# kyungminn/PBHC

Hardware: AMD Instinct MI355X
Metric: env-steps/s (obs+reward+PPO update), 4096 G1 envs @1/2/4/8 MI355X (higher is better)
Workload: dtype f32; 1 GPU; 4096 envs/GPU, G1 23-DoF, single reference motion g1_walk_45cms (122 frames), v1 env (LeggedRobotMotionTracking) + MHPPO, 24 steps/iter, 5 epochs x 4 minibatches; replay sim-stub tensors resident in HBM; envs_per_gpu=4096, global_envs=4096, num_steps_per_env=24, parallelism=dp1

## Files before the change

### pbhc_amd/csrc/pbhc_gemm.hip

```cpp
#include <hip/hip_runtime.h>
#include <stdint.h>
#include <stdio.h>

#include "../../include/pbhc_hip.h"

extern thread_local char g_pbhc_err[512];
#define GEMM_FAIL(code, ...) do { snprintf(g_pbhc_err, sizeof(g_pbhc_err), __VA_ARGS__); return (code); } while (0)
#define GEMM_ARG(cond) do { if (!(cond)) GEMM_FAIL(PBHC_EINVAL, "%s: argument check failed: %s", __func__, #cond); } while (0)
#define GEMM_HIP(expr) do { hipError_t e_ = (expr); if (e_ != hipSuccess) GEMM_FAIL(PBHC_EHIP, "%s: %s: %s", __func__, #expr, hipGetErrorString(e_)); } while (0)

typedef float f32x16 __attribute__((ext_vector_type(16)));
typedef float f32x4 __attribute__((ext_vector_type(4)));
typedef float f32x2 __attribute__((ext_vector_type(2)));

#define GEMM_T 256

#ifndef PBHC_GEMM_LIBM_EXP
#define GEMM_EXP(x) __builtin_amdgcn_exp2f((x) * 1.44269504088896341f)
#define GEMM_RCP(x) __builtin_amdgcn_rcpf(x)
#else
#define GEMM_EXP(x) expf(x)
#define GEMM_RCP(x) (1.0f / (x))
#endif
__device__ __forceinline__ float gemm_act(int act, float v) {
// ... 309 lines not shown
    } else {
      prow_or_kr = 2 * (p - A_PIECES) + (lane >> 5);
      c = ((lane & 31) - 8 * ((prow_or_kr >> 2) & 1)) & 31;
    }
  };
  unsigned voff[LPW];
#pragma unroll
  for (int i = 0; i < LPW; ++i) {
    int q, c; bool kc, isA;
    piece_geom(i, q, c, kc, isA);
    if (kc) {
      const int grow = min((isA ? row0 : col0) + q, (isA ? M : N) - 1);
      voff[i] = ((unsigned)grow * (unsigned)(isA ? lda : K) + 4u * c) * 4u;
    } else {
      voff[i] = ((unsigned)q * (unsigned)N + (unsigned)min(col0 + 4 * c, N - 4)) * 4u;
    }
  }
  auto issue = [&](int st, auto slot_c) {
    constexpr int SLOT = decltype(slot_c)::value;
    const int k0 = st * BK;
    if (tail && st == nk - 1) {
#pragma unroll
      for (int i = 0; i < LPW; ++i) {
        const int p = (wave + 4 * i) % PIECES;
        int q, c; bool kc, isA;
        piece_geom(i, q, c, kc, isA);
        const float* g;
        if (kc) {
          const int grow = min((isA ? row0 : col0) + q, (isA ? M : N) - 1);
          const float* rowbase = (isA ? A : B) + (size_t)grow * (isA ? lda : K);
          const int gk = k0 + 4 * c;
          g = gk + 4 <= K ? rowbase + gk : gk < K ? rowbase + (K - 4) : g_gemm_zeros;
        } else {
          g = k0 + q < K ? B + (size_t)(k0 + q) * N + min(col0 + 4 * c, N - 4) : g_gemm_zeros;
        }
        glds16(g, &lds[SLOT * STAGE + p * 256]);
      }
    } else {
      const char* sA = reinterpret_cast<const char*>(A + k0);
      const char* sB = reinterpret_cast<const char*>(MODE == 0 ? B + k0 : B + (size_t)k0 * N);
#pragma unroll
      for (int i = 0; i < LPW; ++i) {
        const int p = (wave + 4 * i) % PIECES;
        const char* sbase = p < A_PIECES ? sA : sB;
        glds16_sv(sbase, voff[i], &lds[SLOT * STAGE + p * 256]);
      }
    }
  };

  f32x16 acc[TM][TN];
#pragma unroll
  for (int j = 0; j < TN; ++j) {
    const int colj = col0 + (wn * TN + j) * 32 + r;
    const float bj = (MODE == 0 && bias && colj < N) ? bias[colj] : 0.0f;
#pragma unroll
    for (int i = 0; i < TM; ++i)
#pragma unroll
      for (int e = 0; e < 16; ++e) acc[i][j][e] = bj;
  }

  const int sw_r = BK == 16 ? (r >> 2) & 3 : (r >> 1) & 7;
  int fa[BK / 8], fb[MODE == 0 ? BK / 8 : TN];
#pragma unroll
  for (int k8 = 0; k8 < BK / 8; ++k8) {
    fa[k8] = (wm * TM * 32 + r) * BK + 4 * ((2 * k8 + kk) ^ sw_r);
    if (MODE == 0) fb[k8] = A_STAGE + (wn * TN * 32 + r) * BK + 4 * ((2 * k8 + kk) ^ sw_r);
  }
  if (MODE == 1) {
#pragma unroll
    for (int j = 0; j < TN; ++j) fb[j] = A_STAGE + 4 * kk * BN + (((wn * TN + j) * 32 + r + 32 * kk) & 127);
  }

  auto stage_body = [&](auto slot_c, int kb) {
    constexpr int SLOT = decltype(slot_c)::value;
    if (kb + NS - 2 < nk) wait_vmcnt<(NS - 2) * LPW>(); else wait_vmcnt<0>();
    lds_barrier_raw();
    if (kb + NS - 1 < nk && !(dbg & 1)) issue(kb + NS - 1, IC<(SLOT + NS - 1) % NS>{});
    if (tail && kb == nk - 1 && (K & 3)) {
      const int rem = K & 3, cst = (K - ktail0) >> 2;
      const int nrows = MODE == 0 ? BM + BN : BM;
      for (int t = tid; t < nrows; t += GEMM_T) {
        const int sw = BK == 16 ? (t >> 2) & 3 : (t >> 1) & 7;
        f32x4* q = reinterpret_cast<f32x4*>(&lds[SLOT * STAGE + t * BK + 4 * (cst ^ sw)]);
        const f32x4 o = *q;
        f32x4 n;
        n[0] = rem == 1 ? o[3] : rem == 2 ? o[2] : o[1];
        n[1] = rem == 1 ? 0.0f : rem == 2 ? o[3] : o[2];
        n[2] = rem == 3 ? o[3] : 0.0f;
        n[3] = 0.0f;
        *q = n;
      }
      lds_barrier_raw();
    }
    f32x4 a[2][TM], b[2][TN];
    auto read_frags = [&](int k8, f32x4 (&af)[TM], f32x4 (&bf)[TN]) {
#pragma unroll
      for (int i = 0; i < TM; ++i) af[i] = *reinterpret_cast<const f32x4*>(&lds[SLOT * STAGE + i * 32 * BK + fa[k8]]);
#pragma unroll
      for (int j = 0; j < TN; ++j) {
        if (MODE == 0) {
          bf[j] = *reinterpret_cast<const f32x4*>(&lds[SLOT * STAGE + j * 32 * BK + fb[k8]]);
        } else {
#pragma unroll
          for (int s = 0; s < 4; ++s) bf[j][s] = lds[SLOT * STAGE + (k8 * 8 + s) * BN + fb[j]];
        }
      }
    };
    read_frags(0, a[0], b[0]);
#pragma unroll
    for (int k8 = 0; k8 < BK / 8; ++k8) {
      if (k8 + 1 < BK / 8) read_frags(k8 + 1, a[(k8 + 1) & 1], b[(k8 + 1) & 1]);
      __builtin_amdgcn_sched_barrier(0);
#pragma unroll
      for (int s = 0; s < 4; ++s)
#pragma unroll
        for (int i = 0; i < TM; ++i)
#pragma unroll
          for (int j = 0; j < TN; ++j) acc[i][j] = __builtin_amdgcn_mfma_f32_32x32x2f32(a[k8 & 1][i][s], b[k8 & 1][j][s], acc[i][j], 0, 0, 0);
    }
  };

  if (0 < nk) issue(0, IC<0>{});
  if (NS > 2 && 1 < nk) issue(1, IC<1 % NS>{});
  if (NS > 3 && 2 < nk) issue(2, IC<2 % NS>{});
  for (int kb = 0; kb < nk; kb += NS) {
    stage_body(IC<0>{}, kb);
    if (kb + 1 < nk) stage_body(IC<1 % NS>{}, kb + 1);
    if (NS > 2 && kb + 2 < nk) stage_body(IC<2 % NS>{}, kb + 2);
    if (NS > 3 && kb + 3 < nk) stage_body(IC<3 % NS>{}, kb + 3);
  }

  if ((dbg & 16) && acc[0][0][0] != 12345.678f) return;
  constexpr int CS = BN + 4;
  constexpr bool CAN_FUSE_OUT = MODE == 0 && BM == 32 && BN == 128;
  const bool fuse_out = CAN_FUSE_OUT && fo.out != nullptr;
  f32x4 wo[3];
  if (CAN_FUSE_OUT && fuse_out) {
#pragma unroll
    for (int q = 0; q < 3; ++q) {
      const int ch = tid + GEMM_T * q;
      const int n = ch >> 5;
      wo[q] = n < fo.no ? reinterpret_cast<const F4U*>(fo.w + (size_t)n * 128 + 4 * (ch & 31))->v : f32x4{0.f, 0.f, 0.f, 0.f};
    }
  }
  lds_barrier_raw();
  if (CAN_FUSE_OUT && fuse_out) {
#pragma unroll
    for (int q = 0; q < 4; ++q) {
      const int ch = tid + GEMM_T * q;
      const int n = ch >> 5;
      f32x4 v = q < 3 ? wo[q < 3 ? q : 0] : f32x4{0.f, 0.f, 0.f, 0.f};
      if (q == 3 && n < fo.no) v = reinterpret_cast<const F4U*>(fo.w + (size_t)n * 128 + 4 * (ch & 31))->v;
      *reinterpret_cast<f32x4*>(&lds[BM * CS + n * CS + 4 * (ch & 31)]) = v;
    }
  }
#pragma unroll
  for (int i = 0; i < TM; ++i)
#pragma unroll
    for (int j = 0; j < TN; ++j)
#pragma unroll
      for (int e = 0; e < 16; ++e)
        lds[((wm * TM + i) * 32 + 8 * (e >> 2) + 4 * kk + (e & 3)) * CS + (wn * TN + j) * 32 + r] = acc[i][j][e];
  lds_barrier_raw();
  {
    constexpr int RP = GEMM_T / (BN / 4);
    constexpr int NP = BM / RP;
    const int c4 = (tid % (BN / 4)) * 4, rr = tid / (BN / 4);
    const int col = col0 + c4;
    const bool vec = (N & 3) == 0;
    const bool cok = vec ? col < N : col < N;
    float csum[4] = {0.f, 0.f, 0.f, 0.f};
    f32x4 sv[NP];
    if (MODE == 1 && act) {
#pragma unroll
      for (int p = 0; p < NP; ++p) {
        const int row = row0 + p * RP + rr;
        sv[p] = f32x4{0.f, 0.f, 0.f, 0.f};
        if (row < M && cok) {
          const float* sp = S + (size_t)row * N + col;
          if (vec) sv[p] = reinterpret_cast<const F4U*>(sp)->v;
          else {
#pragma unroll
            for (int q = 0; q < 4; ++q) if (col + q < N) sv[p][q] = sp[q];
          }
        }
      }
    }
    auto row_pass = [&](auto act_c, auto vec_c) {
      constexpr int ACT = decltype(act_c)::value;
      constexpr bool VEC = (decltype(vec_c)::value & 1) != 0;
      constexpr bool INTERIOR = (decltype(vec_c)::value & 2) != 0;
#pragma unroll
    for (int p = 0; p < NP; ++p) {
      const int row = row0 + p * RP + rr;
      f32x4 v = *reinterpret_cast<const f32x4*>(&lds[(p * RP + rr) * CS + c4]);
      const bool ok = INTERIOR || (row < M && cok);
      if (MODE == 0) {
        if (Pre && ok) {
          float* pp = Pre + (size_t)row * ldc + col;
          if (VEC) reinterpret_cast<F4U*>(pp)->v = v;
          else {
#pragma unroll
            for (int q = 0; q < 4; ++q) if (col + q < N) pp[q] = v[q];
          }
        }
        v = gemm_act4<ACT>(v);
        if (CAN_FUSE_OUT && fuse_out) *reinterpret_cast<f32x4*>(&lds[(p * RP + rr) * CS + c4]) = v;
      } else if (ACT) {
        v = gemm_mul_grad4<ACT>(v, sv[p]);
      }
      if (ok && !((dbg & 2) && v[0] != 12345.678f)) {
        float* cp = Cout + (size_t)row * ldc + col;
        if (VEC && (dbg & 4)) __builtin_nontemporal_store(v, &reinterpret_cast<F4U*>(cp)->v);
        else if (VEC) reinterpret_cast<F4U*>(cp)->v = v;
        else {
#pragma unroll
          for (int q = 0; q < 4; ++q) if (col + q < N) cp[q] = v[q];
        }
        if (MODE == 1) {
#pragma unroll
          for (int q = 0; q < 4; ++q) csum[q] += v[q];
        }
      }
    }
    };
    const bool interior = row0 + BM <= M && col0 + BN <= N;
    if (vec && interior) {
      if (act == 1) row_pass(IC<1>{}, IC<3>{}); else if (act == 2) row_pass(IC<2>{}, IC<3>{}); else if (act == 3) row_pass(IC<3>{}, IC<3>{}); else row_pass(IC<0>{}, IC<3>{});
    } else if (vec) {
      if (act == 1) row_pass(IC<1>{}, IC<1>{}); else if (act == 2) row_pass(IC<2>{}, IC<1>{}); else if (act == 3) row_pass(IC<3>{}, IC<1>{}); else row_pass(IC<0>{}, IC<1>{});
    } else {
      if (act == 1) row_pass(IC<1>{}, IC<0>{}); else if (act == 2) row_pass(IC<2>{}, IC<0>{}); else if (act == 3) row_pass(IC<3>{}, IC<0>{}); else row_pass(IC<0>{}, IC<0>{});
    }
    if ((dbg & 8) && threadIdx.x == 0 && blockIdx.x == gridDim.x / 2) {
      __builtin_amdgcn_s_waitcnt(0);
      Cout[0] = (float)(clock64() - dbg_c0);
      Cout[1] = (float)(wall_clock64() - dbg_w0);
    }
    if constexpr (CAN_FUSE_OUT) {
      if (fuse_out) {
        lds_barrier_raw();
        f32x16 o;
#pragma unroll
        for (int e = 0; e < 16; ++e) o[e] = 0.0f;
#pragma unroll
        for (int k8 = 0; k8 < 4; ++k8) {
          const f32x4 ya = *reinterpret_cast<const f32x4*>(&lds[r * CS + 32 * wave + 8 * k8 + 4 * kk]);
          const f32x4 wb = *reinterpret_cast<const f32x4*>(&lds[BM * CS + r * CS + 32 * wave + 8 * k8 + 4 * kk]);
#pragma unroll
          for (int s = 0; s < 4; ++s) o = __builtin_amdgcn_mfma_f32_32x32x2f32(ya[s], wb[s], o, 0, 0, 0);
        }
        lds_barrier_raw();
#pragma unroll
        for (int e = 0; e < 16; ++e) lds[wave * (32 * 33) + (8 * (e >> 2) + 4 * kk + (e & 3)) * 33 + r] = o[e];
        lds_barrier_raw();
        const int m = tid >> 3, q0 = tid & 7;
        if (row0 + m < M) {
#pragma unroll
          for (int j = 0; j < 4; ++j) {
            const int n = q0 + 8 * j;
            if (n < fo.no) {
              float t = lds[m * 33 + n];
#pragma unroll
              for (int w = 1; w < 4; ++w) t += lds[w * (32 * 33) + m * 33 + n];
              fo.out[(size_t)(row0 + m) * fo.no + n] = t + (fo.b ? fo.b[n] : 0.0f);
            }
          }
        }
      }
    }
    if (MODE == 1 && part) {
      lds_barrier_raw();
      float* red = lds;
#pragma unroll
      for (int q = 0; q < 4; ++q) red[rr * BN + c4 + q] = csum[q];
      lds_barrier_raw();
      for (int c = tid; c < BN; c += GEMM_T) {
        float t = 0.0f;
#pragma unroll
        for (int w = 0; w < RP; ++w) t += red[w * BN + c];
        if (col0 + c < N) part[(size_t)tile_m * N + col0 + c] = t;
      }
    }
  }
}

template <int MODE, int WM, int WN, int TM, int TN, int BK, int NS>
__global__ __launch_bounds__(GEMM_T, 2) void k_gemm2(const float* __restrict__ A, const float* __restrict__ B, const float* __restrict__ bias,
                                                      const float* __restrict__ S, float* __restrict__ Cout, float* __restrict__ Pre, float* __restrict__ part,
                                                      int M, int N, int K, int act, int tiles_n, int dbg, int lda, int ldc, long long a_batch, long long c_batch,
                                                      GemmOutLayer fo) {
  const size_t ao = (size_t)blockIdx.y * a_batch, co = (size_t)blockIdx.y * c_batch;
  const Gemm2Args g{A + ao, B, bias, S, Cout + co, Pre ? Pre + co : nullptr, part, M, N, K, act, tiles_n, dbg, lda, ldc, fo};
  gemm2_tile<MODE, WM, WN, TM, TN, BK, NS>(g, blockIdx.x, gridDim.x);
}

template <int MODE, int WM, int WN, int TM, int TN, int BK, int NS>
__global__ __launch_bounds__(GEMM_T, 2) void k_gemm2_pair(Gemm2Args g0, Gemm2Args g1, int n0) {
  const bool first = (int)blockIdx.x < n0;
  const Gemm2Args g = first ? g0 : g1;
  gemm2_tile<MODE, WM, WN, TM, TN, BK, NS>(g, first ? blockIdx.x : blockIdx.x - n0, first ? n0 : gridDim.x - n0);
}

#define WG_BK 32
#define WG_BM 128
#define WG_BN 128
__global__ __launch_bounds__(GEMM_T, 2) void k_wgrad(const float* __restrict__ dY, const float* __restrict__ X, float* __restrict__ part,
                                                      int N, int K, int stages_total, int tiles_k, int tiles, int P) {
  constexpr int A_STAGE = WG_BK * WG_BM, STAGE = WG_BK * (WG_BM + WG_BN);
  constexpr int A_PIECES = A_STAGE / 256, PIECES = STAGE / 256, LPW = PIECES / 4;
  extern __shared__ __attribute__((aligned(16))) float lds[];
  int tile, p_idx;
  if ((P & 7) == 0) { const int xcd = blockIdx.x & 7, slot = blockIdx.x >> 3; p_idx = xcd + 8 * (slot / tiles); tile = slot - (slot / tiles) * tiles; }
  else { p_idx = blockIdx.x / tiles; tile = blockIdx.x - p_idx * tiles; }
  const int tile_n = tile / tiles_k, tile_k = tile - tile_n * tiles_k;
  const int n0 = tile_n * WG_BM, k0c = tile_k * WG_BN;
  const int tid = threadIdx.x, lane = tid & 63;
  const int wave = __builtin_amdgcn_readfirstlane(tid >> 6);
  const int wm = wave >> 1, wn = wave & 1;
  const int r = lane & 31, kk = lane >> 5;
  const int st0 = (int)((long long)p_idx * stages_total / P), st1 = (int)((long long)(p_idx + 1) * stages_total / P);
  const int nk = st1 - st0;
  const float* dYp = dY + (size_t)st0 * WG_BK * N;
  const float* Xp = X + (size_t)st0 * WG_BK * K;

  unsigned voff[LPW];
#pragma unroll
  for (int i = 0; i < LPW; ++i) {
    const int p = wave + 4 * i;
    const bool isA = p < A_PIECES;
    const int row = (isA ? p : p - A_PIECES) * 2 + (lane >> 5);
    const int c = lane & 31;
    const int col = isA ? min(n0 + 4 * c, N - 4) : min(k0c + 4 * c, K - 4);
    voff[i] = ((unsigned)row * (unsigned)(isA ? N : K) + (unsigned)col) * 4u;
  }
  auto issue = [&](int st, auto slot_c) {
    constexpr int SLOT = decltype(slot_c)::value;
    const char* sA = reinterpret_cast<const char*>(dYp + (size_t)st * WG_BK * N);
    const char* sB = reinterpret_cast<const char*>(Xp + (size_t)st * WG_BK * K);
#pragma unroll
    for (int i = 0; i < LPW; ++i) {
      const int p = wave + 4 * i;
      glds16_sv(p < A_PIECES ? sA : sB, voff[i], &lds[SLOT * STAGE + p * 256]);
    }
  };

  f32x16 acc[2][2];
#pragma unroll
  for (int q = 0; q < 2; ++q)
#pragma unroll
    for (int p = 0; p < 2; ++p)
#pragma unroll
      for (int e = 0; e < 16; ++e) acc[q][p][e] = 0.0f;
  const int fa = kk * WG_BM + wm * 64 + 2 * r;
  const int fb = A_STAGE + kk * WG_BN + wn * 64 + 2 * r;

  auto stage_body = [&](auto slot_c, int kb) {
    constexpr int SLOT = decltype(slot_c)::value;
    wait_vmcnt<0>();
    lds_barrier_raw();
    if (kb + 1 < nk) issue(kb + 1, IC<(SLOT + 1) % 2>{});
    f32x2 a[2][4], b[2][4];
    auto read_frags = [&](int g, f32x2 (&af)[4], f32x2 (&bf)[4]) {
#pragma unroll
      for (int t = 0; t < 4; ++t) {
        af[t] = *reinterpret_cast<const f32x2*>(&lds[SLOT * STAGE + (8 * g + 2 * t) * WG_BM + fa]);
        bf[t] = *reinterpret_cast<const f32x2*>(&lds[SLOT * STAGE + (8 * g + 2 * t) * WG_BN + fb]);
      }
    };
    read_frags(0, a[0], b[0]);
#pragma unroll
    for (int g = 0; g < WG_BK / 8; ++g) {
      if (g + 1 < WG_BK / 8) read_frags(g + 1, a[(g + 1) & 1], b[(g + 1) & 1]);
      __builtin_amdgcn_sched_barrier(0);
#pragma unroll
      for (int t = 0; t < 4; ++t)
#pragma unroll
        for (int q = 0; q < 2; ++q)
#pragma unroll
          for (int p = 0; p < 2; ++p) acc[q][p] = __builtin_amdgcn_mfma_f32_32x32x2f32(a[g & 1][t][q], b[g & 1][t][p], acc[q][p], 0, 0, 0);
    }
  };
  if (nk > 0) issue(0, IC<0>{});
  for (int kb = 0; kb < nk; kb += 2) {
    stage_body(IC<0>{}, kb);
    if (kb + 1 < nk) stage_body(IC<1>{}, kb + 1);
  }

  constexpr int CS = WG_BN + 4;
  lds_barrier_raw();
#pragma unroll
  for (int q = 0; q < 2; ++q)
#pragma unroll
    for (int e = 0; e < 16; ++e) {
      const int row = wm * 64 + 2 * (8 * (e >> 2) + 4 * kk + (e & 3)) + q;
      *reinterpret_cast<f32x2*>(&lds[row * CS + wn * 64 + 2 * r]) = f32x2{acc[q][0][e], acc[q][1][e]};
    }
  lds_barrier_raw();
  float* out = part + (size_t)p_idx * N * K;
  const int c4 = (tid & 31) * 4, rr = tid >> 5;
  const int col = k0c + c4;
  const int rem = K & 3;
  const bool straddle = rem != 0 && col < K && col + 4 > K;
#pragma unroll
  for (int p = 0; p < WG_BM / 8; ++p) {
    const int row = n0 + p * 8 + rr;
    f32x4 v = *reinterpret_cast<const f32x4*>(&lds[(p * 8 + rr) * CS + c4]);
    if (row < N && col < K) {
      float* cp = out + (size_t)row * K + col;
      if (!straddle) {
        reinterpret_cast<F4U*>(cp)->v = v;
      } else {
        cp[0] = rem == 1 ? v[3] : rem == 2 ? v[2] : v[1];
        if (rem >= 2) cp[1] = rem == 2 ? v[3] : v[2];
        if (rem == 3) cp[2] = v[3];
      }
    }
  }
}

__global__ __launch_bounds__(256) void k_wgrad_sum(const float* __restrict__ part, float* __restrict__ dW, int n, int P) {
  const int i = (blockIdx.x * 256 + threadIdx.x) * 4;
  if (i >= n) return;
  if (i + 4 <= n) {
    f32x4 s = {0.f, 0.f, 0.f, 0.f};
    int p = 0;
    for (; p + 8 <= P; p += 8) {
      f32x4 q[8];
#pragma unroll
      for (int u = 0; u < 8; ++u) q[u] = reinterpret_cast<const F4U*>(part + (size_t)(p + u) * n + i)->v;
#pragma unroll
      for (int u = 0; u < 8; ++u) s += q[u];
    }
    for (; p < P; ++p) s += reinterpret_cast<const F4U*>(part + (size_t)p * n + i)->v;
    reinterpret_cast<F4U*>(dW + i)->v = s;
  } else {
    for (int j = i; j < n; ++j) {
      float s = 0.0f;
      for (int p = 0; p < P; ++p) s += part[(size_t)p * n + j];
      dW[j] = s;
    }
  }
}

static int g_dbg = 0;
template <int MODE, int WM, int WN, int TM, int TN, int BK>
static hipError_t gemm_launch(const float* A, const float* B, const float* bias, const float* S, float* C, float* pre, float* part, int M, int N, int K, int act,
                              hipStream_t st) {
  constexpr int BM = 32 * WM * TM, BN = 32 * WN * TN;
  constexpr int LDS_BYTES = 2 * (BM * (BK + 4) + (MODE == 0 ? BN * (BK + 4) : BK * (BN + 8))) * 4;
  static bool attr_set = LDS_BYTES <= 65536;
  if (!attr_set) {
    hipError_t e = hipFuncSetAttribute(reinterpret_cast<const void*>(&k_gemm<MODE, WM, WN, TM, TN, BK>), hipFuncAttributeMaxDynamicSharedMemorySize, LDS_BYTES);
    if (e != hipSuccess) return e;
    attr_set = true;
  }
  const int tm = (M + BM - 1) / BM, tn = (N + BN - 1) / BN;
  hipLaunchKernelGGL((k_gemm<MODE, WM, WN, TM, TN, BK>), dim3(tm * tn), dim3(GEMM_T), LDS_BYTES, st, A, B, bias, S, C, pre, part, M, N, K, act, tn, g_dbg);
  return hipGetLastError();
}

static int tile_bm(int shape) { return shape == 0 ? 128 : shape == 1 ? 96 : shape == 4 ? 32 : 64; }

template <int MODE, int WM, int WN, int TM, int TN, int BK, int NS>
constexpr int gemm2_lds_bytes() {
  constexpr int BM = 32 * WM * TM, BN = 32 * WN * TN;
  constexpr int RING_BYTES = NS * (BM + BN) * BK * 4, IMAGE_BYTES = (BM + (MODE == 0 && BM == 32 && BN == 128 ? 32 : 0)) * (BN + 4) * 4;
  return RING_BYTES > IMAGE_BYTES ? RING_BYTES : IMAGE_BYTES;
}
template <int MODE, int WM, int WN, int TM, int TN, int BK, int NS>
static hipError_t gemm2_launch(const float* A, const float* B, const float* bias, const float* S, float* C, float* pre, float* part, int M, int N, int K, int act,
                               hipStream_t st, int lda = 0, int ldc = 0, long long a_batch = 0, long long c_batch = 0, int batches = 1,
                               GemmOutLayer fo = GemmOutLayer{nullptr, nullptr, nullptr, 0}) {
  constexpr int BM = 32 * WM * TM, BN = 32 * WN * TN;
  constexpr int LDS_BYTES = gemm2_lds_bytes<MODE, WM, WN, TM, TN, BK, NS>();
  static bool attr_set = LDS_BYTES <= 65536;
  if (!attr_set) {
    hipError_t e = hipFuncSetAttribute(reinterpret_cast<const void*>(&k_gemm2<MODE, WM, WN, TM, TN, BK, NS>), hipFuncAttributeMaxDynamicSharedMemorySize, LDS_BYTES);
    if (e != hipSuccess) return e;
    attr_set = true;
  }
  const int tm = (M + BM - 1) / BM, tn = (N + BN - 1) / BN;
  hipLaunchKernelGGL((k_gemm2<MODE, WM, WN, TM, TN, BK, NS>), dim3(tm * tn, batches), dim3(GEMM_T), LDS_BYTES, st, A, B, bias, S, C, pre, part, M, N, K, act, tn, g_dbg,
                     lda ? lda : K, ldc ? ldc : N, a_batch, c_batch, fo);
  return hipGetLastError();
}

#ifndef PBHC_GEMM_BK
#define PBHC_GEMM_BK 32
#endif
static int g_variant = 0;
template <int MODE, int WM, int WN, int TM, int TN>
static hipError_t gemm_variant(const float* A, const float* B, const float* bias, const float* S, float* C, float* pre, float* part, int M, int N, int K, int act,
                               hipStream_t st) {
  const bool v2ok = K >= 4 && (MODE == 0 || (N & 3) == 0) && (size_t)M * K < (1u << 30) && (size_t)(MODE == 0 ? N : K) * (MODE == 0 ? K : N) < (1u << 30);
  if (g_variant == 1 || !v2ok) return gemm_launch<MODE, WM, WN, TM, TN, PBHC_GEMM_BK>(A, B, bias, S, C, pre, part, M, N, K, act, st);
  if (g_variant == 2) return gemm2_launch<MODE, WM, WN, TM, TN, 16, 3>(A, B, bias, S, C, pre, part, M, N, K, act, st);
  return gemm2_launch<MODE, WM, WN, TM, TN, 32, 2>(A, B, bias, S, C, pre, part, M, N, K, act, st);
}
template <int MODE>
static hipError_t gemm_dispatch(int shape, const float* A, const float* B, const float* bias, const float* S, float* C, float* pre, float* part, int M, int N, int K,
                                int act, hipStream_t st) {
  if (shape == 0) return gemm_variant<MODE, 2, 2, 2, 2>(A, B, bias, S, C, pre, part, M, N, K, act, st);
  if (shape == 1) return gemm_variant<MODE, 1, 4, 3, 1>(A, B, bias, S, C, pre, part, M, N, K, act, st);
  if constexpr (MODE == 0) {
    if (shape == 3) return gemm_variant<MODE, 2, 2, 1, 1>(A, B, bias, S, C, pre, part, M, N, K, act, st);
  }
  if (shape == 4) return gemm_variant<MODE, 1, 4, 1, 1>(A, B, bias, S, C, pre, part, M, N, K, act, st);
  return gemm_variant<MODE, 1, 4, 2, 1>(A, B, bias, S, C, pre, part, M, N, K, act, st);
}

static int pick_shape(int M, int N, int K, int forced, bool forward) {
  if (forced >= 0 && forced <= 4) return forced;
  if (forward && N <= 64) return 3;
  if (M <= 32 * PBHC_ACT_MAX_BLOCKS && M >= 8192 && (forward ? N <= 128 : K <= 128)) return 4;
  if (N <= 128 && M % 96 == 0 && (M / 96) % 256 == 0) return 1;
  if (forward && (long)((M + 63) / 64) * ((N + 127) / 128) < 512) return 3;
  return 2;
}
static int g_force_shape = -1;

extern "C" {

void pbhc_gemm_debug_force_shape(int shape) {
  if (shape < 0) { g_force_shape = -1; g_dbg = 0; g_variant = 0; return; }
  g_force_shape = (shape & 0xff) == 0xff ? -1 : shape & 0xff;
  g_dbg = (shape >> 8) & 0xff;
  g_variant = (shape >> 16) & 0xff;
}

int pbhc_linear_act_fwd(const float* x, const float* w, const float* bias, float* y, float* pre, int M, int N, int K, int act, void* stream) {
  GEMM_ARG(x && w && y && M >= 1 && N >= 1 && K >= 1 && act >= 0 && act <= 3);
  GEMM_ARG(((uintptr_t)x & 3) == 0 && ((uintptr_t)w & 3) == 0);
  GEMM_HIP(gemm_dispatch<0>(pick_shape(M, N, K, g_force_shape, true), x, w, bias, nullptr, y, pre, nullptr, M, N, K, act, (hipStream_t)stream));
  return PBHC_OK;
}

int pbhc_linear_act_fwd_out(const float* x, const float* w, const float* bias, float* y, float* pre, int M, int N, int K, int act, const float* w_out,
                            const float* b_out, int NO, float* out, void* stream) {
  GEMM_ARG(x && w && y && w_out && out && M >= 1 && N == 128 && K >= 4 && NO >= 1 && NO <= 32 && act >= 0 && act <= 3);
  GEMM_ARG(((uintptr_t)x & 3) == 0 && ((uintptr_t)w & 3) == 0 && ((uintptr_t)w_out & 3) == 0);
  GEMM_ARG((size_t)M * K < (1u << 30) && (size_t)N * K < (1u << 30));
  const GemmOutLayer fo{w_out, b_out, out, NO};
  hipStream_t st = (hipStream_t)stream;
  if (g_variant == 2) GEMM_HIP((gemm2_launch<0, 1, 4, 1, 1, 16, 3>(x, w, bias, nullptr, y, pre, nullptr, M, N, K, act, st, 0, 0, 0, 0, 1, fo)));
  else if (g_variant == 3) GEMM_HIP((gemm2_launch<0, 1, 4, 1, 1, 16, 4>(x, w, bias, nullptr, y, pre, nullptr, M, N, K, act, st, 0, 0, 0, 0, 1, fo)));
  else GEMM_HIP((gemm2_launch<0, 1, 4, 1, 1, 32, 2>(x, w, bias, nullptr, y, pre, nullptr, M, N, K, act, st, 0, 0, 0, 0, 1, fo)));
  return PBHC_OK;
}

static int dgrad_shape(int M, int N, int K) {
  int shape = pick_shape(M, N, K, g_force_shape, false);
  if (shape == 3) shape = 2;
  if ((M + tile_bm(shape) - 1) / tile_bm(shape) > PBHC_ACT_MAX_BLOCKS) shape = 0;
  return shape;
}

int pbhc_linear_dgrad_act_pairable(int M, int N, int K) {
  if (M < 1 || N < 1 || K < 1 || g_variant != 0 || g_dbg != 0) return 0;
  const bool v2ok = K >= 4 && (N & 3) == 0 && (size_t)M * K < (1u << 30) && (size_t)K * N < (1u << 30);
  return v2ok && dgrad_shape(M, N, K) == 4;
}

int pbhc_linear_dgrad_act(const float* dy, const float* w, const float* saved, float* dx, float* scratch, int* num_row_blocks, int M, int N, int K,
                          int act, void* stream) {
  GEMM_ARG(dy && w && dx && M >= 1 && N >= 1 && K >= 1 && act >= 0 && act <= 3 && (act == 0 || saved) && (!scratch || num_row_blocks));
  GEMM_ARG(((uintptr_t)dy & 3) == 0 && ((uintptr_t)w & 3) == 0);
  const int shape = dgrad_shape(M, N, K);
  const int nb = (M + tile_bm(shape) - 1) / tile_bm(shape);
  GEMM_ARG(!scratch || nb <= PBHC_ACT_MAX_BLOCKS);
  if (num_row_blocks) *num_row_blocks = nb;
  GEMM_HIP(gemm_dispatch<1>(shape, dy, w, nullptr, saved, dx, nullptr, scratch, M, N, K, act, (hipStream_t)stream));
  return PBHC_OK;
}

}

template <int MODE, int TM>
static hipError_t gemm2_pair_launch(const Gemm2Args& p0, const Gemm2Args& p1, bool swap, hipStream_t st) {
  constexpr int BM = 32 * TM;
  constexpr int LDS_BYTES = gemm2_lds_bytes<MODE, 1, 4, TM, 1, 32, 2>();
  static_assert(LDS_BYTES <= 65536, "no attribute to set");
  const Gemm2Args& a = swap ? p1 : p0;
  const Gemm2Args& b = swap ? p0 : p1;
  const int na = ((a.M + BM - 1) / BM) * a.tiles_n, nb = ((b.M + BM - 1) / BM) * b.tiles_n;
  hipLaunchKernelGGL((k_gemm2_pair<MODE, 1, 4, TM, 1, 32, 2>), dim3(na + nb), dim3(GEMM_T), LDS_BYTES, st, a, b, na);
  return hipGetLastError();
}
static int fwd_out_check(const float* x, const float* w, const float* y, int M, int N, int K, int act, const float* w_out, int NO, const float* out) {
  GEMM_ARG(x && w && y && w_out && out && M >= 1 && N == 128 && K >= 4 && NO >= 1 && NO <= 32 && act >= 0 && act <= 3);
  GEMM_ARG(((uintptr_t)x & 3) == 0 && ((uintptr_t)w & 3) == 0 && ((uintptr_t)w_out & 3) == 0);
  GEMM_ARG((size_t)M * K < (1u << 30) && (size_t)N * K < (1u << 30));
  return PBHC_OK;
}
static int dgrad_pair_check(const float* dy, const float* w, const float* saved, const float* dx, const float* scratch, int* num_row_blocks, int M, int N, int K,
                            int act) {
  GEMM_ARG(dy && w && dx && M >= 1 && N >= 1 && K >= 1 && act >= 0 && act <= 3 && (act == 0 || saved) && (!scratch || num_row_blocks));
  GEMM_ARG(((uintptr_t)dy & 3) == 0 && ((uintptr_t)w & 3) == 0);
  GEMM_ARG(K >= 4 && K <= 128 && (N & 3) == 0 && (size_t)M * K < (1u << 30) && (size_t)K * N < (1u << 30));
  GEMM_ARG(!scratch || (M + 31) / 32 <= PBHC_ACT_MAX_BLOCKS);
  return PBHC_OK;
}

extern "C" {

int pbhc_linear_act_fwd_out_pair(const float* x0, const float* w0, const float* bias0, float* y0, float* pre0, int M0, int N0, int K0, int act0, const float* w_out0,
                                 const float* b_out0, int NO0, float* out0, const float* x1, const float* w1, const float* bias1, float* y1, float* pre1, int M1,
                                 int N1, int K1, int act1, const float* w_out1, const float* b_out1, int NO1, float* out1, void* stream) {
  int rc = fwd_out_check(x0, w0, y0, M0, N0, K0, act0, w_out0, NO0, out0);
  if (rc == PBHC_OK) rc = fwd_out_check(x1, w1, y1, M1, N1, K1, act1, w_out1, NO1, out1);
  if (rc != PBHC_OK) return rc;
  if (g_variant != 0 || g_dbg != 0) {
    rc = pbhc_linear_act_fwd_out(x0, w0, bias0, y0, pre0, M0, N0, K0, act0, w_out0, b_out0, NO0, out0, stream);
    return rc != PBHC_OK ? rc : pbhc_linear_act_fwd_out(x1, w1, bias1, y1, pre1, M1, N1, K1, act1, w_out1, b_out1, NO1, out1, stream);
  }
  const Gemm2Args p0{x0, w0, bias0, nullptr, y0, pre0, nullptr, M0, N0, K0, act0, 1, 0, K0, N0, GemmOutLayer{w_out0, b_out0, out0, NO0}};
  const Gemm2Args p1{x1, w1, bias1, nullptr, y1, pre1, nullptr, M1, N1, K1, act1, 1, 0, K1, N1, GemmOutLayer{w_out1, b_out1, out1, NO1}};
  GEMM_HIP((gemm2_pair_launch<0, 1>(p0, p1, K1 > K0, (hipStream_t)stream)));
  return PBHC_OK;
}

int pbhc_linear_dgrad_act_pair(const float* dy0, const float* w0, const float* saved0, float* dx0, float* scratch0, int* num_row_blocks0, int M0, int N0, int K0,
                               int act0, const float* dy1, const float* w1, const float* saved1, float* dx1, float* scratch1, int* num_row_blocks1, int M1, int N1,
                               int K1, int act1, void* stream) {
  int rc = dgrad_pair_check(dy0, w0, saved0, dx0, scratch0, num_row_blocks0, M0, N0, K0, act0);
  if (rc == PBHC_OK) rc = dgrad_pair_check(dy1, w1, saved1, dx1, scratch1, num_row_blocks1, M1, N1, K1, act1);
  if (rc != PBHC_OK) return rc;
  GEMM_ARG(g_variant == 0 && g_dbg == 0);
  if (num_row_blocks0) *num_row_blocks0 = (M0 + 31) / 32;
  if (num_row_blocks1) *num_row_blocks1 = (M1 + 31) / 32;
  const GemmOutLayer none{nullptr, nullptr, nullptr, 0};
  const Gemm2Args p0{dy0, w0, nullptr, saved0, dx0, nullptr, scratch0, M0, N0, K0, act0, (N0 + 127) / 128, 0, K0, N0, none};
  const Gemm2Args p1{dy1, w1, nullptr, saved1, dx1, nullptr, scratch1, M1, N1, K1, act1, (N1 + 127) / 128, 0, K1, N1, none};
  GEMM_HIP((gemm2_pair_launch<1, 1>(p0, p1, (size_t)N1 * K1 > (size_t)N0 * K0, (hipStream_t)stream)));
  return PBHC_OK;
}

int pbhc_linear_act_fwd_pairable(int M, int N, int K) {
  if (M < 1 || N < 1 || K < 1 || g_variant != 0 || g_dbg != 0) return 0;
  const bool v2ok = K >= 4 && (size_t)M * K < (1u << 30) && (size_t)N * K < (1u << 30);
  return v2ok && pick_shape(M, N, K, g_force_shape, true) == 2;
}

int pbhc_linear_act_fwd_pair(const float* x0, const float* w0, const float* bias0, float* y0, float* pre0, int M0, int N0, int K0, int act0, const float* x1,
                             const float* w1, const float* bias1, float* y1, float* pre1, int M1, int N1, int K1, int act1, void* stream) {
  GEMM_ARG(x0 && w0 && y0 && M0 >= 1 && N0 >= 1 && K0 >= 1 && act0 >= 0 && act0 <= 3 && ((uintptr_t)x0 & 3) == 0 && ((uintptr_t)w0 & 3) == 0);
  GEMM_ARG(x1 && w1 && y1 && M1 >= 1 && N1 >= 1 && K1 >= 1 && act1 >= 0 && act1 <= 3 && ((uintptr_t)x1 & 3) == 0 && ((uintptr_t)w1 & 3) == 0);
  GEMM_ARG(pbhc_linear_act_fwd_pairable(M0, N0, K0) && pbhc_linear_act_fwd_pairable(M1, N1, K1));
  const GemmOutLayer none{nullptr, nullptr, nullptr, 0};
  const int tn0 = (N0 + 127) / 128, tn1 = (N1 + 127) / 128;
  const Gemm2Args p0{x0, w0, bias0, nullptr, y0, pre0, nullptr, M0, N0, K0, act0, tn0, 0, K0, N0, none};
  const Gemm2Args p1{x1, w1, bias1, nullptr, y1, pre1, nullptr, M1, N1, K1, act1, tn1, 0, K1, N1, none};
  const size_t work0 = (size_t)((M0 + 63) / 64) * tn0 * K0, work1 = (size_t)((M1 + 63) / 64) * tn1 * K1;
  GEMM_HIP((gemm2_pair_launch<0, 2>(p0, p1, work1 > work0, (hipStream_t)stream)));
  return PBHC_OK;
}


int pbhc_linear_act_fwd_strided(const float* x, int lda, long long x_batch_stride, const float* w, const float* bias, float* y, float* pre, int ldc,
                                long long y_batch_stride, int batches, int M, int N, int K, int act, void* stream) {
  GEMM_ARG(x && w && y && M >= 1 && N >= 1 && K >= 4 && act >= 0 && act <= 3 && lda >= K && ldc >= N && batches >= 1 && batches <= 65535);
  GEMM_ARG(((uintptr_t)x & 3) == 0 && ((uintptr_t)w & 3) == 0 && x_batch_stride >= 0 && y_batch_stride >= 0);
  GEMM_ARG((size_t)M * (size_t)lda < (1u << 30) && (size_t)N * (size_t)K < (1u << 30));
  hipStream_t st = (hipStream_t)stream;
  const int shape = pick_shape(M, N, K, g_force_shape, true);
  hipError_t e;
  if (shape == 3) e = gemm2_launch<0, 2, 2, 1, 1, 32, 2>(x, w, bias, nullptr, y, pre, nullptr, M, N, K, act, st, lda, ldc, x_batch_stride, y_batch_stride, batches);
  else if (shape == 1) e = gemm2_launch<0, 1, 4, 3, 1, 32, 2>(x, w, bias, nullptr, y, pre, nullptr, M, N, K, act, st, lda, ldc, x_batch_stride, y_batch_stride, batches);
  else if (shape == 0) e = gemm2_launch<0, 2, 2, 2, 2, 32, 2>(x, w, bias, nullptr, y, pre, nullptr, M, N, K, act, st, lda, ldc, x_batch_stride, y_batch_stride, batches);
  else e = gemm2_launch<0, 1, 4, 2, 1, 32, 2>(x, w, bias, nullptr, y, pre, nullptr, M, N, K, act, st, lda, ldc, x_batch_stride, y_batch_stride, batches);
  GEMM_HIP(e);
  return PBHC_OK;
}

int pbhc_linear_wgrad_parts(int M, int N, int K) {
  if (M < 32 || (M & 31) || N < 4 || (N & 3) || K < 4) return 0;
  const int tiles = ((N + WG_BM - 1) / WG_BM) * ((K + WG_BN - 1) / WG_BN);
  const int stages = M / WG_BK;
  int P = 512 / tiles;
  if (P > stages / 4) P = stages / 4;
  if (P > 256) P = 256;
  if (P >= 8 && (P & ~7) * 10 >= P * 9) P &= ~7;
  return P < 1 ? 1 : P;
}

int pbhc_linear_wgrad(const float* dy, const float* x, float* dw, float* scratch, int M, int N, int K, void* stream) {
  GEMM_ARG(dy && x && dw && scratch && M >= 1 && N >= 1 && K >= 1);
  GEMM_ARG(((uintptr_t)dy & 3) == 0 && ((uintptr_t)x & 3) == 0);
  const int P = pbhc_linear_wgrad_parts(M, N, K);
  GEMM_ARG(P >= 1 && (M & 31) == 0 && (N & 3) == 0 && K >= 4 && (size_t)M * (size_t)(N > K ? N : K) < (1u << 30));
  hipStream_t st = (hipStream_t)stream;
  const int tn = (N + WG_BM - 1) / WG_BM, tk = (K + WG_BN - 1) / WG_BN;
  constexpr int RING = 2 * WG_BK * (WG_BM + WG_BN) * 4, IMAGE = WG_BM * (WG_BN + 4) * 4;
  constexpr int LDS_BYTES = RING > IMAGE ? RING : IMAGE;
  static bool attr_set = false;
  if (!attr_set) {
    GEMM_HIP(hipFuncSetAttribute(reinterpret_cast<const void*>(&k_wgrad), hipFuncAttributeMaxDynamicSharedMemorySize, LDS_BYTES));
    attr_set = true;
  }
  hipLaunchKernelGGL(k_wgrad, dim3(tn * tk * P), dim3(GEMM_T), LDS_BYTES, st, dy, x, scratch, N, K, M / WG_BK, tk, tn * tk, P);
  const int n = N * K;
  hipLaunchKernelGGL(k_wgrad_sum, dim3((n / 4 + 256) / 256), dim3(256), 0, st, scratch, dw, n, P);
  GEMM_HIP(hipGetLastError());
  return PBHC_OK;
}

}
```

Measured before the change: 3.218 million env-steps/s.

## Add persistent warp-specialized dgrad kernel with LDS-resident weights for K=128

```diff
diff --git a/pbhc_amd/csrc/pbhc_gemm.hip b/pbhc_amd/csrc/pbhc_gemm.hip
--- a/pbhc_amd/csrc/pbhc_gemm.hip
+++ b/pbhc_amd/csrc/pbhc_gemm.hip
@@ -635,6 +635,157 @@
   gemm2_tile<MODE, WM, WN, TM, TN, BK, NS>(g, first ? blockIdx.x : blockIdx.x - n0, first ? n0 : gridDim.x - n0);
 }
 
+#define WS_T 512
+constexpr int WS_W_FLOATS = 128 * 128, WS_DY_FLOATS = 32 * 128, WS_CS = 132, WS_IMG_FLOATS = 32 * WS_CS, WS_RED_FLOATS = 8 * 128;
+constexpr int WS_TEAM_FLOATS = WS_DY_FLOATS + WS_IMG_FLOATS + WS_RED_FLOATS;
+constexpr int WS_LDS_BYTES = (WS_W_FLOATS + 2 * WS_TEAM_FLOATS) * 4;
+
+__device__ __forceinline__ f32x4 gload16_sv(const void* sbase, unsigned voff) {
+  f32x4 v;
+  asm volatile("global_load_dwordx4 %0, %1, %2" : "=&v"(v) : "v"(voff), "s"(sbase) : "memory");
+  return v;
+}
+
+__global__ __launch_bounds__(WS_T) void k_dgrad_ws(Gemm2Args g0, Gemm2Args g1, int n0) {
+  extern __shared__ __attribute__((aligned(16))) float lds[];
+  const bool first = (int)blockIdx.x < n0;
+  const Gemm2Args g = first ? g0 : g1;
+  const float* __restrict__ A = g.A;
+  const float* __restrict__ B = g.B;
+  const float* __restrict__ S = g.S;
+  float* __restrict__ Cout = g.Cout;
+  float* __restrict__ part = g.part;
+  const int M = g.M, N = g.N, act = g.act, tn = g.tiles_n;
+  int b = first ? (int)blockIdx.x : (int)blockIdx.x - n0;
+  const int G = first ? n0 : (int)gridDim.x - n0;
+  const int q = G / tn, rem = G - q * tn;
+  int slice, wi, gs;
+  if (b < rem * (q + 1)) { slice = b / (q + 1); wi = b - slice * (q + 1); gs = q + 1; }
+  else { b -= rem * (q + 1); slice = rem + b / q; wi = b - (slice - rem) * q; gs = q; }
+  const int tiles_m = (M + 31) >> 5;
+  const int per = tiles_m / gs, extra = tiles_m - per * gs;
+  const int t0 = wi * per + min(wi, extra), cnt = per + (wi < extra ? 1 : 0);
+  if (cnt == 0) return;
+  const int col0 = slice * 128;
+
+  const int tid = threadIdx.x, lane = tid & 63, ltid = tid & 255;
+  const int wave = __builtin_amdgcn_readfirstlane(tid >> 6);
+  const int team = wave >> 2, wn = wave & 3;
+  const int r = lane & 31, kk = lane >> 5;
+  float* Wl = lds;
+  float* dyb = lds + WS_W_FLOATS + team * WS_TEAM_FLOATS;
+  float* img = dyb + WS_DY_FLOATS;
+  float* red = img + WS_IMG_FLOATS;
+
+#pragma unroll
+  for (int i = 0; i < 8; ++i) {
+    const int bp = wave + 8 * i;
+    const int kr = 2 * bp + kk;
+    const int c = ((lane & 31) - 8 * ((kr >> 2) & 1)) & 31;
+    glds16_sv(B, ((unsigned)kr * (unsigned)N + (unsigned)min(col0 + 4 * c, N - 4)) * 4u, Wl + bp * 256);
+  }
+  const int dy_row = wn * 8 + (lane >> 3);
+  const int dy_c = (lane & 7) ^ ((dy_row >> 1) & 7);
+  auto issue_dy = [&](int tile) {
+    const int row0 = tile * 32;
+    const char* sb = reinterpret_cast<const char*>(A + (size_t)row0 * 128);
+    const unsigned vo = ((unsigned)min(dy_row, M - 1 - row0) * 128u + 4u * dy_c) * 4u;
+#pragma unroll
+    for (int i = 0; i < 4; ++i) glds16_sv(sb, vo + 128u * i, dyb + (4 * i + wn) * 256);
+  };
+  if (team < cnt) issue_dy(t0 + team);
+
+  const int sw_r = (r >> 1) & 7;
+  int fa[4];
+#pragma unroll
+  for (int k8 = 0; k8 < 4; ++k8) fa[k8] = r * 32 + 4 * ((2 * k8 + kk) ^ sw_r);
+  const int fb = 4 * kk * 128 + ((wn * 32 + r + 32 * kk) & 127);
+  const int c4 = (ltid & 31) * 4, rr = ltid >> 5;
+  const bool cok = col0 + c4 < N;
+
+  f32x16 acc;
+  f32x4 sv[4], fra[2], frb[2];
+#pragma unroll
+  for (int e = 0; e < 16; ++e) acc[e] = 0.0f;
+#pragma unroll
+  for (int p = 0; p < 4; ++p) sv[p] = f32x4{0.f, 0.f, 0.f, 0.f};
+  fra[0] = fra[1] = frb[0] = frb[1] = f32x4{0.f, 0.f, 0.f, 0.f};
+
+  auto read_frags = [&](int kb, f32x4& af, f32x4& bf) {
+    af = *reinterpret_cast<const f32x4*>(&dyb[(kb >> 2) * 1024 + fa[kb & 3]]);
+#pragma unroll
+    for (int s = 0; s < 4; ++s) bf[s] = Wl[(kb * 8 + s) * 128 + fb];
+  };
+  auto mfma_blocks = [&](auto half_c) {
+    constexpr int K0 = decltype(half_c)::value * 8;
+#pragma unroll
+    for (int kb = K0; kb < K0 + 8; ++kb) {
+      if (kb + 1 < 16) read_frags(kb + 1, fra[(kb + 1) & 1], frb[(kb + 1) & 1]);
+      __builtin_amdgcn_sched_barrier(0);
+#pragma unroll
+      for (int s = 0; s < 4; ++s) acc = __builtin_amdgcn_mfma_f32_32x32x2f32(fra[kb & 1][s], frb[kb & 1][s], acc, 0, 0, 0);
+    }
+  };
+
+  for (int h = 0; h <= cnt; ++h) {
+    const bool mf = h < cnt && (h & 1) == team;
+    const bool ep = h >= 1 && ((h - 1) & 1) == team;
+    float csum[4] = {0.f, 0.f, 0.f, 0.f};
+    wait_vmcnt<0>();
+    asm volatile("" : "+v"(sv[0]), "+v"(sv[1]), "+v"(sv[2]), "+v"(sv[3]));
+    if (ep) {
+#pragma unroll
+      for (int e = 0; e < 16; ++e) img[(8 * (e >> 2) + 4 * kk + (e & 3)) * WS_CS + wn * 32 + r] = acc[e];
+    }
+    lds_barrier_raw();
+    if (mf) {
+      const int row0 = (t0 + h) * 32;
+      if (act) {
+        const char* sb = reinterpret_cast<const char*>(S + (size_t)row0 * N + col0);
+#pragma unroll
+        for (int p = 0; p < 4; ++p)
+          sv[p] = gload16_sv(sb, ((unsigned)min(p * 8 + rr, M - 1 - row0) * (unsigned)N + (unsigned)min(c4, N - 4 - col0)) * 4u);
+      }
+#pragma unroll
+      for (int e = 0; e < 16; ++e) acc[e] = 0.0f;
+      read_frags(0, fra[0], frb[0]);
+      mfma_blocks(IC<0>{});
+    }
+    if (ep) {
+      if (h + 1 < cnt) issue_dy(t0 + h + 1);
+      const int row0 = (t0 + h - 1) * 32;
+      const int col = col0 + c4;
+      auto row_pass = [&](auto act_c) {
+        constexpr int ACT = decltype(act_c)::value;
+#pragma unroll
+        for (int p = 0; p < 4; ++p) {
+          const int row = row0 + p * 8 + rr;
+          f32x4 v = *reinterpret_cast<const f32x4*>(&img[(p * 8 + rr) * WS_CS + c4]);
+          if (ACT) v = gemm_mul_grad4<ACT>(v, sv[p]);
+          if (row < M && cok) {
+            reinterpret_cast<F4U*>(Cout + (size_t)row * N + col)->v = v;
+#pragma unroll
+            for (int qq = 0; qq < 4; ++qq) csum[qq] += v[qq];
+          }
+        }
+      };
+      if (act == 1) row_pass(IC<1>{}); else if (act == 2) row_pass(IC<2>{}); else if (act == 3) row_pass(IC<3>{}); else row_pass(IC<0>{});
+      if (part) {
+#pragma unroll
+        for (int qq = 0; qq < 4; ++qq) red[rr * 128 + c4 + qq] = csum[qq];
+      }
+    }
+    lds_barrier_raw();
+    if (mf) mfma_blocks(IC<1>{});
+    if (ep && part && ltid < 128) {
+      float t = 0.0f;
+#pragma unroll
+      for (int w = 0; w < 8; ++w) t += red[w * 128 + ltid];
+      if (col0 + ltid < N) part[(size_t)(t0 + h - 1) * N + col0 + ltid] = t;
+    }
+  }
+}
+
 #define WG_BK 32
 #define WG_BM 128
 #define WG_BN 128
@@ -853,13 +1004,48 @@
 }
 static int g_force_shape = -1;
 
+static bool variant_plain() { return g_variant == 0 || g_variant == 4; }
+static int g_ws_wgs = 0;
+static int g_ws_cus = 0;
+static hipError_t dgrad_ws_init() {
+  if (g_ws_cus > 0) return hipSuccess;
+  hipError_t e = hipFuncSetAttribute(reinterpret_cast<const void*>(&k_dgrad_ws), hipFuncAttributeMaxDynamicSharedMemorySize, WS_LDS_BYTES);
+  if (e != hipSuccess) return e;
+  int dev = 0, cus = 0;
+  if ((e = hipGetDevice(&dev)) != hipSuccess) return e;
+  if ((e = hipDeviceGetAttribute(&cus, hipDeviceAttributeMultiprocessorCount, dev)) != hipSuccess) return e;
+  g_ws_cus = cus > 0 ? cus : 256;
+  return hipSuccess;
+}
+static bool dgrad_ws_applies(int M, int N, int K) {
+  return K == 128 && g_variant == 0 && g_dbg == 0;
+}
+static hipError_t dgrad_ws_launch(const Gemm2Args& p0, const Gemm2Args* p1, hipStream_t st) {
+  hipError_t e = dgrad_ws_init();
+  if (e != hipSuccess) return e;
+  const long long w0 = (long long)((p0.M + 31) / 32) * p0.tiles_n, w1 = p1 ? (long long)((p1->M + 31) / 32) * p1->tiles_n : 0;
+  const int slices = p0.tiles_n + (p1 ? p1->tiles_n : 0);
+  long long G = g_ws_wgs > 0 ? g_ws_wgs : g_ws_cus;
+  if (G > w0 + w1) G = w0 + w1;
+  if (G < slices) G = slices;
+  long long G0 = G;
+  if (p1) {
+    G0 = (G * w0 + (w0 + w1) / 2) / (w0 + w1);
+    if (G0 < p0.tiles_n) G0 = p0.tiles_n;
+    if (G0 > G - p1->tiles_n) G0 = G - p1->tiles_n;
+  }
+  hipLaunchKernelGGL(k_dgrad_ws, dim3((unsigned)G), dim3(WS_T), WS_LDS_BYTES, st, p0, p1 ? *p1 : p0, (int)G0);
+  return hipGetLastError();
+}
+
 extern "C" {
 
 void pbhc_gemm_debug_force_shape(int shape) {
-  if (shape < 0) { g_force_shape = -1; g_dbg = 0; g_variant = 0; return; }
+  if (shape < 0) { g_force_shape = -1; g_dbg = 0; g_variant = 0; g_ws_wgs = 0; return; }
   g_force_shape = (shape & 0xff) == 0xff ? -1 : shape & 0xff;
   g_dbg = (shape >> 8) & 0xff;
   g_variant = (shape >> 16) & 0xff;
+  g_ws_wgs = (shape >> 24) & 0x7f;
 }
 
 int pbhc_linear_act_fwd(const float* x, const float* w, const float* bias, float* y, float* pre, int M, int N, int K, int act, void* stream) {
@@ -890,9 +1076,11 @@
 }
 
 int pbhc_linear_dgrad_act_pairable(int M, int N, int K) {
-  if (M < 1 || N < 1 || K < 1 || g_variant != 0 || g_dbg != 0) return 0;
+  if (M < 1 || N < 1 || K < 1 || !variant_plain() || g_dbg != 0) return 0;
   const bool v2ok = K >= 4 && (N & 3) == 0 && (size_t)M * K < (1u << 30) && (size_t)K * N < (1u << 30);
-  return v2ok && dgrad_shape(M, N, K) == 4;
+  if (!(v2ok && dgrad_shape(M, N, K) == 4)) return 0;
+  if (dgrad_ws_applies(M, N, K)) (void)dgrad_ws_init();
+  return 1;
 }
 
 int pbhc_linear_dgrad_act(const float* dy, const float* w, const float* saved, float* dx, float* scratch, int* num_row_blocks, int M, int N, int K,
@@ -903,6 +1091,12 @@
   const int nb = (M + tile_bm(shape) - 1) / tile_bm(shape);
   GEMM_ARG(!scratch || nb <= PBHC_ACT_MAX_BLOCKS);
   if (num_row_blocks) *num_row_blocks = nb;
+  const bool v2ok = K >= 4 && (N & 3) == 0 && (size_t)M * K < (1u << 30) && (size_t)K * N < (1u << 30);
+  if (shape == 4 && v2ok && dgrad_ws_applies(M, N, K)) {
+    const Gemm2Args p{dy, w, nullptr, saved, dx, nullptr, scratch, M, N, K, act, (N + 127) / 128, 0, K, N, GemmOutLayer{nullptr, nullptr, nullptr, 0}};
+    GEMM_HIP(dgrad_ws_launch(p, nullptr, (hipStream_t)stream));
+    return PBHC_OK;
+  }
   GEMM_HIP(gemm_dispatch<1>(shape, dy, w, nullptr, saved, dx, nullptr, scratch, M, N, K, act, (hipStream_t)stream));
   return PBHC_OK;
 }
@@ -943,7 +1137,7 @@
   int rc = fwd_out_check(x0, w0, y0, M0, N0, K0, act0, w_out0, NO0, out0);
   if (rc == PBHC_OK) rc = fwd_out_check(x1, w1, y1, M1, N1, K1, act1, w_out1, NO1, out1);
   if (rc != PBHC_OK) return rc;
-  if (g_variant != 0 || g_dbg != 0) {
+  if (!variant_plain() || g_dbg != 0) {
     rc = pbhc_linear_act_fwd_out(x0, w0, bias0, y0, pre0, M0, N0, K0, act0, w_out0, b_out0, NO0, out0, stream);
     return rc != PBHC_OK ? rc : pbhc_linear_act_fwd_out(x1, w1, bias1, y1, pre1, M1, N1, K1, act1, w_out1, b_out1, NO1, out1, stream);
   }
@@ -959,18 +1153,20 @@
   int rc = dgrad_pair_check(dy0, w0, saved0, dx0, scratch0, num_row_blocks0, M0, N0, K0, act0);
   if (rc == PBHC_OK) rc = dgrad_pair_check(dy1, w1, saved1, dx1, scratch1, num_row_blocks1, M1, N1, K1, act1);
   if (rc != PBHC_OK) return rc;
-  GEMM_ARG(g_variant == 0 && g_dbg == 0);
+  GEMM_ARG(variant_plain() && g_dbg == 0);
   if (num_row_blocks0) *num_row_blocks0 = (M0 + 31) / 32;
   if (num_row_blocks1) *num_row_blocks1 = (M1 + 31) / 32;
   const GemmOutLayer none{nullptr, nullptr, nullptr, 0};
   const Gemm2Args p0{dy0, w0, nullptr, saved0, dx0, nullptr, scratch0, M0, N0, K0, act0, (N0 + 127) / 128, 0, K0, N0, none};
   const Gemm2Args p1{dy1, w1, nullptr, saved1, dx1, nullptr, scratch1, M1, N1, K1, act1, (N1 + 127) / 128, 0, K1, N1, none};
-  GEMM_HIP((gemm2_pair_launch<1, 1>(p0, p1, (size_t)N1 * K1 > (size_t)N0 * K0, (hipStream_t)stream)));
+  const bool swap = (size_t)N1 * K1 > (size_t)N0 * K0;
+  if (dgrad_ws_applies(M0, N0, K0) && dgrad_ws_applies(M1, N1, K1)) GEMM_HIP(dgrad_ws_launch(swap ? p1 : p0, swap ? &p0 : &p1, (hipStream_t)stream));
+  else GEMM_HIP((gemm2_pair_launch<1, 1>(p0, p1, swap, (hipStream_t)stream)));
   return PBHC_OK;
 }
 
 int pbhc_linear_act_fwd_pairable(int M, int N, int K) {
-  if (M < 1 || N < 1 || K < 1 || g_variant != 0 || g_dbg != 0) return 0;
+  if (M < 1 || N < 1 || K < 1 || !variant_plain() || g_dbg != 0) return 0;
   const bool v2ok = K >= 4 && (size_t)M * K < (1u << 30) && (size_t)N * K < (1u << 30);
   return v2ok && pick_shape(M, N, K, g_force_shape, true) == 2;
 }
```

New measurement: 3.286 million env-steps/s, median of 6. 1.02x the previous value.
